# entn-at/exemplars_vc

Hardware: AMD Instinct MI355X
Metric: spectral frames/sec converted (100 NMF iters, N=4096 dict) (higher is better)
Workload: dtype f64

## Files before the change

exemplars_vc_amd/csrc/evc_fused_all.hip:

```cpp
#include "evc_fused_common.h"

namespace evc {

constexpr int AW = 4;
constexpr int AKT = 8;
constexpr int ATILES = AW * AKT;
constexpr int ATHREADS = 2 * AW * 64;
constexpr unsigned ALL_POLL_LIMIT = 1u << 17;
#ifndef EVC_ALL_STAGGER_PER_ITER
#define EVC_ALL_STAGGER_PER_ITER 11000
#endif
#ifndef EVC_ALL_EXCH_PRIO
#define EVC_ALL_EXCH_PRIO 3
#endif
#ifndef EVC_ALL_C1_ALTERNATE
#define EVC_ALL_C1_ALTERNATE 0
#endif

constexpr long ALL_LDS_BUDGET = 160 * 1024 - 256;
__host__ __device__ constexpr int all_dict_row(int e) { return 4 * (((e >> 2) & 1) * 2 + (e >> 3)) + (e & 3); }
template <int MSTEPS, int C, bool KL>
struct AllShape {
    static constexpr int MT = MSTEPS > 4 ? 2 : 1;
    static constexpr int E = MT * 4 * 64;
    static constexpr int NE = MSTEPS * 64;
    static constexpr int RSTR = NE < 256 ? 256 : NE;
    static constexpr int STG = C > 0 ? 1 : (C == 0 ? NE : NE + ALL_MAX_MEMBERS - 1);
    static constexpr long REST = 8L * 2 * (AW * RSTR + 2 * E + (KL ? E : 1) + STG) + 3 * 4;
    static constexpr long dict_bytes(int pr) { return 8L * ATILES * 16 * pr; }
    static constexpr int PR_ALL = 4 * MSTEPS + 2;
    static constexpr int PR = KL ? 0
                              : REST + dict_bytes(PR_ALL) <= ALL_LDS_BUDGET       ? PR_ALL
                              : REST + dict_bytes(PR_ALL - 4) <= ALL_LDS_BUDGET   ? PR_ALL - 4
                                                                                  : 0;
    static constexpr bool LDS_DICT = C != 1 && PR > 0 && PR - 1 >= 4 * MSTEPS - 3;
};

#ifdef EVC_ALL_TIMING
#define EVC_STAMP(i)                                                                                             \
    do {                                                                                                         \
        if (a.dbg && tt0 == g - half && lane == 0 && w == 0)                                                     \
            a.dbg[(((long)blockIdx.x * 2 + half) * (2 * a.iters + 1) + step) * 4 + (i)] = __builtin_amdgcn_s_memtime(); \
    } while (0)
#else
#define EVC_STAMP(i)
#endif

template <int MSTEPS, int C, bool KL>
__global__ __launch_bounds__(ATHREADS, 2) void k_fused_all(FusedArgs a) {
    using S = AllShape<MSTEPS, C, KL>;
    constexpr int MT = S::MT;
    constexpr int E = S::E;
    constexpr int NE = S::NE;
    constexpr int RSTR = S::RSTR;
    constexpr int MSP = (MSTEPS + 1) & ~1;
    constexpr int PR = S::PR;
    constexpr int TPD = 16 * PR;
    __shared__ double s_red[2][AW * RSTR];
    __shared__ double s_v[2][E];
    __shared__ double s_x[2][E];
    __shared__ double s_r[2][KL ? E : 1];
    __shared__ double s_stage[2][S::STG];
    __shared__ double s_dict[S::LDS_DICT ? ATILES * TPD : 1];
    __shared__ unsigned s_hb[2];
    __shared__ int s_fail;
    const int tid = threadIdx.x, lane = tid & 63;
    const int w8 = __builtin_amdgcn_readfirstlane(tid >> 6);
    const int half = w8 >> 2, w = w8 & 3, th = tid & (AW * 64 - 1);
    const int CR = C > 0 ? C : a.coop_c;
    const int member = blockIdx.x % CR;
    const int g = 2 * (blockIdx.x / CR) + half;
    double* const red = s_red[half];
    double* const vL = s_v[half];
    double* const xL = s_x[half];
    double* const rL = s_r[half];
    double* const stage = s_stage[half];
    unsigned hb = 0;
    const double* __restrict__ A1p = a.A1p;
    const double* __restrict__ A2p = a.A2p;
    f64x2* __restrict__ Hp = a.Hp;
    const int NT = a.NT;
    const long tile0 = (long)member * ATILES + w;
    const unsigned ul = (unsigned)lane;
    long sw = 0;

    const __amdgpu_buffer_rsrc_t r1 = __builtin_amdgcn_make_buffer_rsrc(const_cast<double*>(A1p), 0, NT * (MSP * 512), 0x00020000);
    const __amdgpu_buffer_rsrc_t r2 = __builtin_amdgcn_make_buffer_rsrc(const_cast<double*>(A2p), 0, NT * (MT * 2048), 0x00020000);
#ifdef EVC_ALL_NOFRAG
    bool nofrag_go = false;
#endif
    const unsigned ul16 = ul * 16u, ul8 = ul * 8u;
    constexpr int BL = 16 * ((MSTEPS - 1) >> 2) + 4 * ((MSTEPS - 1) & 3);
    const int rowA = w * AKT * TPD + all_dict_row(4 * (lane & 3) + ((lane & 15) >> 2)) * PR;
    const int rowB = w * AKT * TPD + all_dict_row(4 * (lane >> 4)) * PR;
    const double* const dA = s_dict + rowA + (lane >> 4);
    const double* const dAL = s_dict + rowA + min(lane >> 4, a.M - BL);
    const double* const dB = s_dict + rowB + (lane & 15);
    const double* const dBL = s_dict + rowB + min(lane & 15, a.M - 16 * (MT - 1));
#define LDS_NO_PAIR() asm volatile("" ::: "memory")
    auto load_a1 = [&](double (&a1)[MSTEPS], int k, auto lds) {
        if constexpr (decltype(lds)::value) {
#pragma unroll
            for (int s = 0; s < MSTEPS; ++s) {
                a1[s] = (s == MSTEPS - 1 ? dAL : dA)[k * TPD + 16 * (s >> 2) + 4 * (s & 3)];
                LDS_NO_PAIR();
            }
            return;
        }
#ifdef EVC_ALL_NOFRAG
        if (nofrag_go) return;
#endif
        const int so = (int)(tile0 + sw + AW * k) * (MSP * 512);
#pragma unroll
        for (int s = 0; s < MSTEPS; s += 2) {
            if (s + 1 < MSTEPS) {
                const f64x2 v = __builtin_bit_cast(f64x2, __builtin_amdgcn_raw_buffer_load_b128(r1, ul16 + (s >> 1) * 1024, so, 0));
                a1[s] = v[0];
                a1[s + 1] = v[1];
            } else {
                a1[s] = __builtin_bit_cast(double, __builtin_amdgcn_raw_buffer_load_b64(r1, ul16 + (s >> 1) * 1024, so, 0));
            }
        }
    };
    auto load_a2 = [&](double (&a2)[MT][4], int k, auto lds) {
        if constexpr (decltype(lds)::value) {
#pragma unroll
            for (int u = 0; u < MT; ++u)
#pragma unroll
                for (int r = 0; r < 4; ++r) {
                    a2[u][r] = (u == MT - 1 ? dBL : dB)[k * TPD + r * PR + 16 * u];
                    LDS_NO_PAIR();
                }
            return;
        }
#ifdef EVC_ALL_NOFRAG
        if (nofrag_go) return;
#endif
        const int so = (int)(tile0 + sw + AW * k) * (MT * 2048);
#pragma unroll
        for (int u = 0; u < MT; ++u)
#pragma unroll
            for (int r = 0; r < 4; r += 2) {
                const f64x2 v = __builtin_bit_cast(f64x2, __builtin_amdgcn_raw_buffer_load_b128(r2, ul16 + (u * 2 + (r >> 1)) * 1024, so, 0));
                a2[u][r] = v[0];
                a2[u][r + 1] = v[1];
            }
    };
    (void)ul8;

    const int mode = a.eps_mode;
    const double eps = a.eps;
    const double d0 = a.l1 + (mode == EVC_EPS_ADD ? a.eps : 0.0);
    const f64x4 dinit = {d0, d0, d0, d0};
    const unsigned lo = fast_lo(mode, eps);
    unsigned seq = 0;
    int rs_es = 1, rs_len = 0, rs_pub0 = 0, rs_pub1 = 0, rs_src0 = -1, rs_src1 = -1, rs_src2 = -1;
    if (C < 0) {
        rs_es = (NE + CR - 1) / CR;
        rs_len = NE - member * rs_es;
        rs_len = rs_len < 0 ? 0 : (rs_len > rs_es ? rs_es : rs_len);
        const int e0 = th, e1 = th + AW * 64;
        const int j0 = e0 / rs_es, j1 = (e1 < NE ? e1 : e0) / rs_es;
        rs_pub0 = (j0 * CR + member) * rs_es + (e0 - j0 * rs_es);
        rs_pub1 = (j1 * CR + member) * rs_es + ((e1 < NE ? e1 : e0) - j1 * rs_es);
        auto src = [&](int idx) {
            if (idx >= CR * rs_es) return -1;
            const int el = idx % rs_es;
            return el < rs_len ? member * CR * rs_es + idx : -1;
        };
        rs_src0 = src(th);
        rs_src1 = src(th + AW * 64);
        rs_src2 = src(th + 2 * AW * 64);
    }
    if (tid == 0) s_fail = 0;
    if (tid < 2) s_hb[tid] = 0;

    if (a.stagger_cycles > 0 && ((blockIdx.x / CR) & 1)) {
        const long long t0 = __builtin_amdgcn_s_memtime();
        while (__builtin_amdgcn_s_memtime() - t0 < a.stagger_cycles) __builtin_amdgcn_s_sleep(32);
    }

    auto run = [&](auto lds) __attribute__((always_inline)) {
    for (long tt0 = g - half; tt0 < a.TT; tt0 += a.groups) {
        const long tt = tt0 + half;
        bool valid;
        {
            const long t = 16 * tt + (lane & 15);
            int u = -1;
            if (tt < a.TT && t < a.T_) u = a.frame_utt[t];
            const bool live = tt < a.TT && ((t >= a.T_) || ((u >= 0) && (a.active[u] != 0)));
            const int v0 = __syncthreads_and(half == 0 ? live : true);
            const int v1 = __syncthreads_and(half == 1 ? live : true);
            valid = (half ? v1 : v0) != 0;
        }
        HTile h[AKT];
        f64x4 p[AKT];
        double a1[MSTEPS], a2[MT][4];
        if (valid && a.first && a.init_const) {
            auto h0_of = [&](int fr) {
                const long t = 16 * tt + fr;
                const int u = t < a.T_ ? a.frame_utt[t] : -1;
                return u >= 0 ? a.h0[u] : 0.0;
            };
            for (int e = th; e < E; e += AW * 64) {
                const int s = e >> 6, l = e & 63;
                const bool in = s < MSTEPS;
                xL[e] = in ? a.Xp[(tt * MSTEPS + s) * 64 + l] : 0.0;
                vL[e] = in ? a.rsum[bin_of(s, l >> 4)] * h0_of(l & 15) : 0.0;
                if (KL) rL[e] = xL[e] / (vL[e] < a.eps ? a.eps : vL[e]);
            }
            const double hv = h0_of(lane & 15);
#pragma unroll
            for (int k = 0; k < AKT; ++k) {
                const long n0 = 16 * (tile0 + AW * k) + 4 * (lane >> 4);
#pragma unroll
                for (int r = 0; r < 4; ++r) h[k][r] = n0 + r < a.N ? hv : 0.0;
            }
        } else if (valid) {
            for (int e = th; e < E; e += AW * 64) {
                const int s = e >> 6, l = e & 63;
                const bool in = s < MSTEPS;
                xL[e] = in ? a.Xp[(tt * MSTEPS + s) * 64 + l] : 0.0;
                vL[e] = in ? a.Vp[(tt * 8 + s) * 64 + l] : 0.0;
                if (KL) rL[e] = xL[e] / (vL[e] < a.eps ? a.eps : vL[e]);
            }
#pragma unroll
            for (int k = 0; k < AKT; ++k) {
                const f64x2* t = Hp + (tt * NT + tile0 + AW * k) * 128;
                const f64x2 h01 = t[ul], h23 = t[ul + 64];
                h[k][0] = h01[0]; h[k][1] = h01[1]; h[k][2] = h23[0]; h[k][3] = h23[1];
            }
        }
        __syncthreads();
        if (valid && !KL) {
            double x[MSTEPS];
#pragma unroll
            for (int s = 0; s < MSTEPS; ++s) x[s] = xL[s * 64 + lane];
            load_a1(a1, 0, lds);
#pragma unroll
            for (int k = 0; k < AKT; ++k) {
                f64x4 acc = {0, 0, 0, 0};
#pragma unroll
                for (int s = 0; s < MSTEPS; ++s) acc = Mma<double>::mma(a1[s], x[s], acc);
                if (!decltype(lds)::value || k + 1 < AKT) load_a1(a1, (k + 1) % AKT, lds);
                p[k] = acc;
            }
        }

        if (valid && KL) load_a1(a1, 0, lds);
        for (int step = 0; step <= 2 * a.iters; ++step) {
#ifdef EVC_ALL_NOFRAG
            nofrag_go = step > 2;
#endif
            const bool mine = (C == 1 && !EVC_ALL_C1_ALTERNATE) ? (step & 1) == 0 : (step & 1) == half;
            EVC_STAMP(0);
            if (valid && mine && step < 2 * a.iters) {
                asm volatile("" : "+s"(sw));
                double v[MSTEPS];
#pragma unroll
                for (int s = 0; s < MSTEPS; ++s) v[s] = KL ? rL[s * 64 + lane] : vL[s * 64 + lane];
                if constexpr (decltype(lds)::value) load_a1(a1, 0, lds);
                f64x4 vn[MT];
#pragma unroll
                for (int u = 0; u < MT; ++u) vn[u] = f64x4{0, 0, 0, 0};
#pragma unroll
                for (int k = 0; k < AKT; ++k) {
                    __builtin_amdgcn_sched_barrier(0);
                    load_a2(a2, k, lds);
                    f64x4 d = KL ? f64x4{0, 0, 0, 0} : dinit;
#pragma unroll
                    for (int s = 0; s < MSTEPS; ++s) d = Mma<double>::mma(a1[s], v[s], d);
                    if (!decltype(lds)::value || k + 1 < AKT)
                        load_a1(a1, (k + 1) % AKT, lds);
                    __builtin_amdgcn_sched_barrier(0);
                    if (KL) {
#pragma unroll
                        for (int r = 0; r < 4; ++r) h[k][r] *= d[r];
                    } else {
                        mu_tile_guarded(h[k], p[k], d, mode, eps, lo);
                    }
#pragma unroll
                    for (int u = 0; u < MT; ++u)
#pragma unroll
                        for (int r = 0; r < 4; ++r) vn[u] = Mma<double>::mma(a2[u][r], h[k][r], vn[u]);
                }
#pragma unroll
                for (int u = 0; u < MT; ++u)
#pragma unroll
                    for (int r = 0; r < 4; ++r)
                        if (u * 4 + r < MSTEPS) red[w * RSTR + (u * 4 + r) * 64 + lane] = vn[u][r];
            } else if (valid && !mine && step > 0) {
                const int e0 = C <= 0 ? th % NE : th, e1 = th + AW * 64;
                const bool has1 = e1 < NE;
                __builtin_amdgcn_s_setprio(EVC_ALL_EXCH_PRIO);
                double s0 = 0.0, s1 = 0.0;
#pragma unroll
                for (int ww = 0; ww < AW; ++ww) {
                    s0 += red[ww * RSTR + e0];
                    s1 += red[ww * RSTR + (has1 ? e1 : e0)];
                }
                if (C < 0) {
                    long long* xb1 = reinterpret_cast<long long*>(a.coop_buf) +
                                     ((size_t)(seq & 1) * a.groups + g) * (size_t)CR * ALL_RS_STRIDE;
                    long long* xb2 = reinterpret_cast<long long*>(a.coop_buf) + ALL_SLICE_OFFSET +
                                     ((size_t)(seq & 1) * a.groups + g) * 512;
                    const long long tag = (seq >> 1) & 1;
                    __hip_atomic_store(xb1 + rs_pub0, (__double_as_longlong(s0) & ~1LL) | tag, __ATOMIC_RELAXED,
                                       __HIP_MEMORY_SCOPE_AGENT);
                    if (has1)
                        __hip_atomic_store(xb1 + rs_pub1, (__double_as_longlong(s1) & ~1LL) | tag, __ATOMIC_RELAXED,
                                           __HIP_MEMORY_SCOPE_AGENT);
                    bool ok = true;
                    auto fetch3 = [&](const long long* p0, const long long* p1, const long long* p2, long long& b0,
                                      long long& b1, long long& b2) {
                        unsigned polls = 0;
                        for (;;) {
                            b0 = __hip_atomic_load(p0, __ATOMIC_RELAXED, __HIP_MEMORY_SCOPE_AGENT);
                            b1 = __hip_atomic_load(p1, __ATOMIC_RELAXED, __HIP_MEMORY_SCOPE_AGENT);
                            b2 = __hip_atomic_load(p2, __ATOMIC_RELAXED, __HIP_MEMORY_SCOPE_AGENT);
                            if (__all(!ok || (((b0 ^ tag) | (b1 ^ tag) | (b2 ^ tag)) & 1) == 0)) break;
                            if (++polls > ALL_POLL_LIMIT ||
                                ((polls & 63) == 0 &&
                                 __hip_atomic_load(a.coop_abort, __ATOMIC_RELAXED, __HIP_MEMORY_SCOPE_AGENT) != 0))
                                ok = false;
                            __builtin_amdgcn_s_sleep(1);
                        }
                    };
                    {
                        long long b0, b1, b2;
                        const long long* own = xb1 + rs_pub0;
                        fetch3(rs_src0 >= 0 ? xb1 + rs_src0 : own, rs_src1 >= 0 ? xb1 + rs_src1 : own,
                               rs_src2 >= 0 ? xb1 + rs_src2 : own, b0, b1, b2);
                        if (rs_src0 >= 0) stage[th] = __longlong_as_double(b0 & ~1LL);
                        if (rs_src1 >= 0) stage[th + AW * 64] = __longlong_as_double(b1 & ~1LL);
                        if (rs_src2 >= 0) stage[th + 2 * AW * 64] = __longlong_as_double(b2 & ~1LL);
                        hb += AW;
                        if (lane == 0)
                            __hip_atomic_fetch_add(&s_hb[half], 1u, __ATOMIC_RELEASE, __HIP_MEMORY_SCOPE_WORKGROUP);
                        while ((int)(__hip_atomic_load(&s_hb[half], __ATOMIC_ACQUIRE, __HIP_MEMORY_SCOPE_WORKGROUP) - hb) < 0)
                            __builtin_amdgcn_s_sleep(1);
                        const int q = th & 3;
                        for (int el = th >> 2; el < rs_len; el += AW * 16) {
                            double v = 0.0;
                            for (int m = q; m < CR; m += 4) v += stage[m * rs_es + el];
                            v += __shfl_xor(v, 1, 64);
                            v += __shfl_xor(v, 2, 64);
                            if (q == 0)
                                __hip_atomic_store(xb2 + member * rs_es + el, (__double_as_longlong(v) & ~1LL) | tag,
                                                   __ATOMIC_RELAXED, __HIP_MEMORY_SCOPE_AGENT);
                        }
                    }
                    long long g0, g1, g2;
                    fetch3(xb2 + e0, xb2 + (has1 ? e1 : e0), xb2 + e0, g0, g1, g2);
                    s0 = __longlong_as_double(g0 & ~1LL);
                    s1 = __longlong_as_double(g1 & ~1LL);
                    ++seq;
                    if (!ok) s_fail = 1;
                } else if (C == 0) {
                    const int ES = NE / CR;
                    long long* xb1 = reinterpret_cast<long long*>(a.coop_buf) +
                                     ((size_t)(seq & 1) * a.groups + g) * (size_t)CR * 512;
                    long long* xb2 = reinterpret_cast<long long*>(a.coop_buf) + ALL_SLICE_OFFSET +
                                     ((size_t)(seq & 1) * a.groups + g) * 512;
                    const long long tag = (seq >> 1) & 1;
                    {
                        const int j0 = e0 / ES, j1 = (has1 ? e1 : e0) / ES;
                        __hip_atomic_store(xb1 + ((size_t)j0 * CR + member) * ES + (e0 - j0 * ES),
                                           (__double_as_longlong(s0) & ~1LL) | tag, __ATOMIC_RELAXED,
                                           __HIP_MEMORY_SCOPE_AGENT);
                        if (has1)
                            __hip_atomic_store(xb1 + ((size_t)j1 * CR + member) * ES + (e1 - j1 * ES),
                                               (__double_as_longlong(s1) & ~1LL) | tag, __ATOMIC_RELAXED,
                                               __HIP_MEMORY_SCOPE_AGENT);
                    }
                    bool ok = true;
                    auto fetch2 = [&](const long long* p0, const long long* p1, long long& b0, long long& b1) {
                        unsigned polls = 0;
                        for (;;) {
                            b0 = __hip_atomic_load(p0, __ATOMIC_RELAXED, __HIP_MEMORY_SCOPE_AGENT);
                            b1 = __hip_atomic_load(p1, __ATOMIC_RELAXED, __HIP_MEMORY_SCOPE_AGENT);
                            if (__all(!ok || (((b0 ^ tag) | (b1 ^ tag)) & 1) == 0)) break;
                            if (++polls > ALL_POLL_LIMIT ||
                                ((polls & 63) == 0 &&
                                 __hip_atomic_load(a.coop_abort, __ATOMIC_RELAXED, __HIP_MEMORY_SCOPE_AGENT) != 0))
                                ok = false;
                            __builtin_amdgcn_s_sleep(1);
                        }
                    };
                    {
                        long long b0, b1;
                        const long long* mine_ = xb1 + (size_t)member * NE;
                        fetch2(mine_ + e0, mine_ + (has1 ? e1 : e0), b0, b1);
                        stage[e0] = __longlong_as_double(b0 & ~1LL);
                        if (has1) stage[e1] = __longlong_as_double(b1 & ~1LL);
                        hb += AW;
                        if (lane == 0)
                            __hip_atomic_fetch_add(&s_hb[half], 1u, __ATOMIC_RELEASE, __HIP_MEMORY_SCOPE_WORKGROUP);
                        while ((int)(__hip_atomic_load(&s_hb[half], __ATOMIC_ACQUIRE, __HIP_MEMORY_SCOPE_WORKGROUP) - hb) < 0)
                            __builtin_amdgcn_s_sleep(1);
                        if (th < 4 * ES) {
                            const int el = th >> 2, q = th & 3, per = CR >> 2;
                            double v = 0.0;
                            for (int i = 0; i < per; ++i) v += stage[(q * per + i) * ES + el];
                            v += __shfl_xor(v, 1, 64);
                            v += __shfl_xor(v, 2, 64);
                            if (q == 0)
                                __hip_atomic_store(xb2 + member * ES + el, (__double_as_longlong(v) & ~1LL) | tag,
                                                   __ATOMIC_RELAXED, __HIP_MEMORY_SCOPE_AGENT);
                        }
                    }
                    long long g0, g1;
                    fetch2(xb2 + e0, xb2 + (has1 ? e1 : e0), g0, g1);
                    s0 = __longlong_as_double(g0 & ~1LL);
                    s1 = __longlong_as_double(g1 & ~1LL);
                    ++seq;
                    if (!ok) s_fail = 1;
                } else if (C > 1) {
                    long long* xb = reinterpret_cast<long long*>(a.coop_buf) +
                                    ((size_t)(seq & 1) * a.groups + g) * (size_t)(C * 512);
                    const long long tag = (seq >> 1) & 1;
                    const long long m0 = (__double_as_longlong(s0) & ~1LL) | tag;
                    const long long m1 = (__double_as_longlong(s1) & ~1LL) | tag;
                    __hip_atomic_store(xb + member * 512 + e0, m0, __ATOMIC_RELAXED, __HIP_MEMORY_SCOPE_AGENT);
                    if (has1) __hip_atomic_store(xb + member * 512 + e1, m1, __ATOMIC_RELAXED, __HIP_MEMORY_SCOPE_AGENT);
                    bool ok = true;
                    unsigned polls = 0;
                    {
                        const long long* sp = xb + (lane < C ? lane : 0) * 512 + (NE - 1);
                        for (;;) {
                            const long long b = __hip_atomic_load(sp, __ATOMIC_RELAXED, __HIP_MEMORY_SCOPE_AGENT);
                            const bool ready = lane >= C || lane == member || (b & 1) == tag;
                            if (__all(ready)) break;
                            if (++polls > ALL_POLL_LIMIT ||
                                ((polls & 63) == 0 &&
                                 __hip_atomic_load(a.coop_abort, __ATOMIC_RELAXED, __HIP_MEMORY_SCOPE_AGENT) != 0)) {
                                ok = false;
                                break;
                            }
                            __builtin_amdgcn_s_sleep(2);
                        }
                    }
                    long long b0[C > 0 ? C : 1] = {}, b1[C > 0 ? C : 1] = {};
                    polls = 0;
                    while (ok) {
#pragma unroll
                        for (int m = 0; m < C; ++m)
                            b0[m] = __hip_atomic_load(xb + m * 512 + e0, __ATOMIC_RELAXED, __HIP_MEMORY_SCOPE_AGENT);
#pragma unroll
                        for (int m = 0; m < C; ++m)
                            b1[m] = __hip_atomic_load(xb + m * 512 + (has1 ? e1 : e0), __ATOMIC_RELAXED, __HIP_MEMORY_SCOPE_AGENT);
                        long long bad = 0;
#pragma unroll
                        for (int m = 0; m < C; ++m) {
                            b0[m] = (m == member) ? m0 : b0[m];
                            b1[m] = (m == member) ? m1 : b1[m];
                            bad |= (b0[m] ^ tag) | (b1[m] ^ tag);
                        }
                        if ((bad & 1) == 0) break;
                        if (++polls > ALL_POLL_LIMIT ||
                            ((polls & 63) == 0 &&
                             __hip_atomic_load(a.coop_abort, __ATOMIC_RELAXED, __HIP_MEMORY_SCOPE_AGENT) != 0)) {
                            ok = false;
                            break;
                        }
                        __builtin_amdgcn_s_sleep(2);
                    }
                    s0 = 0.0; s1 = 0.0;
#pragma unroll
                    for (int m = 0; m < C; ++m) {
                        s0 += __longlong_as_double(b0[m] & ~1LL);
                        s1 += __longlong_as_double(b1[m] & ~1LL);
                    }
                    ++seq;
                    if (!ok) s_fail = 1;
                }
                vL[e0] = s0;
                if (has1) vL[e1] = s1;
                if (KL) {
                    rL[e0] = xL[e0] / (s0 < a.eps ? a.eps : s0);
                    if (has1) rL[e1] = xL[e1] / (s1 < a.eps ? a.eps : s1);
                }
                __builtin_amdgcn_s_setprio(0);
            }
            EVC_STAMP(1);
            __syncthreads();
            EVC_STAMP(2);
            if (C != 1 && s_fail) {
                if (tid == 0) __hip_atomic_store(a.coop_abort, 1, __ATOMIC_RELAXED, __HIP_MEMORY_SCOPE_AGENT);
                return;
            }
        }

        if (valid) {
#pragma unroll
            for (int k = 0; k < AKT; ++k) {
                f64x2* t = Hp + (tt * NT + tile0 + AW * k) * 128;
                t[ul] = f64x2{h[k][0], h[k][1]};
                t[ul + 64] = f64x2{h[k][2], h[k][3]};
            }
            if (a.Hx) {
                const long t = 16 * tt + (lane & 15);
                if (t < a.T_) {
#pragma unroll
                    for (int k = 0; k < AKT; ++k) {
                        const long n0 = 16 * (tile0 + AW * k) + 4 * (lane >> 4);
#pragma unroll
                        for (int r = 0; r < 4; ++r)
                            if (n0 + r < a.N) {
                                if (a.hx_frame_major) a.Hx[t * a.ldhx + n0 + r] = h[k][r];
                                else a.Hx[(n0 + r) * a.ldhx + t] = h[k][r];
                            }
                    }
                }
            }
            if (member == 0) {
                for (int e = th; e < NE; e += AW * 64) a.Vp[(tt * 8 + (e >> 6)) * 64 + (e & 63)] = vL[e];
                if (a.write_err && w == 0) {
                    double e = 0.0;
#pragma unroll
                    for (int s = 0; s < MSTEPS; ++s) {
                        const double x = xL[s * 64 + lane], vv = vL[s * 64 + lane];
                        e += KL ? kl_terms(x, vv, a.eps) : (x - vv) * (x - vv);
                    }
                    e += __shfl_xor(e, 16, 64);
                    e += __shfl_xor(e, 32, 64);
                    const long t = 16 * tt + lane;
                    if (lane < 16 && t < a.T_) a.err2[t] = e;
                }
            }
        }
        __syncthreads();
    }
    };

    if constexpr (S::LDS_DICT) {
        if (a.M > 0 && a.M < PR) {
            for (int x = tid; x < ATILES * TPD; x += ATHREADS) {
                const int slot = x / TPD, e = all_dict_row((x / PR) % 16), b = x % PR;
                const long j = (long)member * ATILES + slot / AKT + AW * (slot % AKT);
                const int q = e >> 2, r = e & 3;
                s_dict[x] = b < a.M ? A2p[((j * MT + (b >> 4)) * 2 + (r >> 1)) * 128 + (16 * q + (b & 15)) * 2 + (r & 1)] : 0.0;
            }
            __syncthreads();
            run(std::true_type{});
            return;
        }
    }
    run(std::false_type{});
}

template <int MSTEPS, int C, bool KL>
static hipError_t launch_all(FusedArgs a, int n_cus, hipStream_t s) {
    int occ = 0;
    hipError_t e = hipOccupancyMaxActiveBlocksPerMultiprocessor(&occ, k_fused_all<MSTEPS, C, KL>, ATHREADS, 0);
    if (e != hipSuccess) return e;
    if (occ < 1) return hipErrorInvalidValue;
    long resident = n_cus;
    if (2 * resident > ALL_MAX_WGS) resident = ALL_MAX_WGS / 2;
    const int cr = C > 0 ? C : a.coop_c;
    if (C == 0 && (cr < 8 || cr > 64 || (cr & (cr - 1)))) return hipErrorInvalidValue;
    if (C < 0 && (cr < 2 || cr > ALL_MAX_MEMBERS)) return hipErrorInvalidValue;
    int pairs = (int)(resident / cr);
    const int want = (a.TT + 1) / 2;
    if (pairs > want) pairs = want;
    if (pairs < 1) return hipErrorInvalidValue;
    a.groups = 2 * pairs;
    a.stagger_cycles = (a.iters > 0 && a.iters <= 25 && a.TT >= 4L * a.groups && pairs >= 2) ? (long long)a.iters * EVC_ALL_STAGGER_PER_ITER : 0;
    if (C != 1) {
        e = hipMemsetAsync(a.coop_buf, 0xFF, sizeof(double) * 2 * (size_t)a.groups * cr * (C < 0 ? ALL_RS_STRIDE : 512), s);
        if (e != hipSuccess) return e;
    }
    if (C <= 0) {
        if (2L * a.groups * 512 > ALL_SLICE_ELEMS) return hipErrorInvalidValue;
        e = hipMemsetAsync(a.coop_buf + ALL_SLICE_OFFSET, 0xFF, sizeof(double) * 2 * (size_t)a.groups * 512, s);
        if (e != hipSuccess) return e;
    }
    hipLaunchKernelGGL((k_fused_all<MSTEPS, C, KL>), dim3((unsigned)(pairs * cr)), dim3(ATHREADS), 0, s, a);
    return hipGetLastError();
}

template <int MSTEPS, bool KL>
static hipError_t pick_c(const FusedArgs& a, int n_cus, hipStream_t s) {
    switch (a.NT / ATILES) {
        case 1: return launch_all<MSTEPS, 1, KL>(a, n_cus, s);
        case 2: return launch_all<MSTEPS, 2, KL>(a, n_cus, s);
        case 4: return launch_all<MSTEPS, 4, KL>(a, n_cus, s);
        case 8:
            if constexpr (AllShape<MSTEPS, 8, KL>::LDS_DICT)
                if (a.M > 0 && a.M < AllShape<MSTEPS, 8, KL>::PR) return launch_all<MSTEPS, 8, KL>(a, n_cus, s);
            return launch_all<MSTEPS, 0, KL>(a, n_cus, s);
        case 16:
        case 32:
        case 64: return launch_all<MSTEPS, 0, KL>(a, n_cus, s);
        default: return launch_all<MSTEPS, -1, KL>(a, n_cus, s);
    }
}

int fused_all_members(int NT, int N, int eps_mode, int exact_div, int loss) {
    if (eps_mode == EVC_EPS_NONE || exact_div || (loss != EVC_LOSS_FROBENIUS && loss != EVC_LOSS_KL)) return 0;
    if (NT % ATILES) return 0;
    const int c = NT / ATILES;
    if (loss == EVC_LOSS_KL && c >= 2 && c < 16) return 0;
    return (c >= 1 && c <= ALL_MAX_MEMBERS) ? c : 0;
}

hipError_t fused_all_launch(int msteps, const FusedArgs& a, int n_cus, hipStream_t s) {
    if (a.NT % ATILES || !a.coop_buf || !a.coop_abort) return hipErrorInvalidValue;
    switch (msteps) {
        case 1: return a.loss == EVC_LOSS_KL ? pick_c<1, true>(a, n_cus, s) : pick_c<1, false>(a, n_cus, s);
        case 2: return a.loss == EVC_LOSS_KL ? pick_c<2, true>(a, n_cus, s) : pick_c<2, false>(a, n_cus, s);
        case 3: return a.loss == EVC_LOSS_KL ? pick_c<3, true>(a, n_cus, s) : pick_c<3, false>(a, n_cus, s);
        case 4: return a.loss == EVC_LOSS_KL ? pick_c<4, true>(a, n_cus, s) : pick_c<4, false>(a, n_cus, s);
        case 5: return a.loss == EVC_LOSS_KL ? pick_c<5, true>(a, n_cus, s) : pick_c<5, false>(a, n_cus, s);
        case 6: return a.loss == EVC_LOSS_KL ? pick_c<6, true>(a, n_cus, s) : pick_c<6, false>(a, n_cus, s);
        case 7: return a.loss == EVC_LOSS_KL ? pick_c<7, true>(a, n_cus, s) : pick_c<7, false>(a, n_cus, s);
        case 8: return a.loss == EVC_LOSS_KL ? pick_c<8, true>(a, n_cus, s) : pick_c<8, false>(a, n_cus, s);
        default: return hipErrorInvalidValue;
    }
}

}
```

Baseline: 1.096 million.

## Restructure cross-block reduction polling and move failure check before barrier

Replaces the two-phase cooperative exchange wait (first spin on a sentinel element, then reload every member's data) with a single loop. Each peer's values are fetched directly, and only peers that have not yet arrived are re-polled, tracked in a bitmask. The failure flag becomes double-buffered per step parity and is read before the barrier, so the post-barrier shared-memory check and the extra serialization it caused go away. It also adds tunable fetch-delay and retry-sleep macros and extra timing stamps; the trade-off is more complex abort semantics, where the early return depends on the previous step's flag.

```diff
diff --git a/exemplars_vc_amd/csrc/evc_fused_all.hip b/exemplars_vc_amd/csrc/evc_fused_all.hip
--- a/exemplars_vc_amd/csrc/evc_fused_all.hip
+++ b/exemplars_vc_amd/csrc/evc_fused_all.hip
@@ -15,6 +15,12 @@
 #endif
 #ifndef EVC_ALL_C1_ALTERNATE
 #define EVC_ALL_C1_ALTERNATE 0
+#endif
+#ifndef EVC_ALL_FETCH_DELAY
+#define EVC_ALL_FETCH_DELAY 0
+#endif
+#ifndef EVC_ALL_RETRY_SLEEP
+#define EVC_ALL_RETRY_SLEEP 2
 #endif
 
 constexpr long ALL_LDS_BUDGET = 160 * 1024 - 256;
@@ -40,7 +46,7 @@
 #define EVC_STAMP(i)                                                                                             \
     do {                                                                                                         \
         if (a.dbg && tt0 == g - half && lane == 0 && w == 0)                                                     \
-            a.dbg[(((long)blockIdx.x * 2 + half) * (2 * a.iters + 1) + step) * 4 + (i)] = __builtin_amdgcn_s_memtime(); \
+            a.dbg[(((long)blockIdx.x * 2 + half) * (2 * a.iters + 1) + step) * 8 + (i)] = __builtin_amdgcn_s_memtime(); \
     } while (0)
 #else
 #define EVC_STAMP(i)
@@ -63,7 +69,7 @@
     __shared__ double s_stage[2][S::STG];
     __shared__ double s_dict[S::LDS_DICT ? ATILES * TPD : 1];
     __shared__ unsigned s_hb[2];
-    __shared__ int s_fail;
+    __shared__ int s_fail[2];
     const int tid = threadIdx.x, lane = tid & 63;
     const int w8 = __builtin_amdgcn_readfirstlane(tid >> 6);
     const int half = w8 >> 2, w = w8 & 3, th = tid & (AW * 64 - 1);
@@ -172,13 +178,18 @@
         rs_src1 = src(th + AW * 64);
         rs_src2 = src(th + 2 * AW * 64);
     }
-    if (tid == 0) s_fail = 0;
+    if (tid < 2) s_fail[tid] = 0;
     if (tid < 2) s_hb[tid] = 0;
 
     if (a.stagger_cycles > 0 && ((blockIdx.x / CR) & 1)) {
         const long long t0 = __builtin_amdgcn_s_memtime();
         while (__builtin_amdgcn_s_memtime() - t0 < a.stagger_cycles) __builtin_amdgcn_s_sleep(32);
     }
+
+    auto give_up = [&](int step) {
+        __hip_atomic_store(a.coop_abort, 1, __ATOMIC_RELAXED, __HIP_MEMORY_SCOPE_AGENT);
+        s_fail[step & 1] = 1;
+    };
 
     auto run = [&](auto lds) __attribute__((always_inline)) {
     for (long tt0 = g - half; tt0 < a.TT; tt0 += a.groups) {
@@ -254,6 +265,12 @@
 #endif
             const bool mine = (C == 1 && !EVC_ALL_C1_ALTERNATE) ? (step & 1) == 0 : (step & 1) == half;
             EVC_STAMP(0);
+            int failed = 0;
+            if (C != 1) {
+                int slot = (step + 1) & 1;
+                asm volatile("" : "+v"(slot));
+                failed = __hip_atomic_load(&s_fail[slot], __ATOMIC_RELAXED, __HIP_MEMORY_SCOPE_WORKGROUP);
+            }
             if (valid && mine && step < 2 * a.iters) {
                 asm volatile("" : "+s"(sw));
                 double v[MSTEPS];
@@ -355,7 +372,7 @@
                     s0 = __longlong_as_double(g0 & ~1LL);
                     s1 = __longlong_as_double(g1 & ~1LL);
                     ++seq;
-                    if (!ok) s_fail = 1;
+                    if (!ok) give_up(step);
                 } else if (C == 0) {
                     const int ES = NE / CR;
                     long long* xb1 = reinterpret_cast<long long*>(a.coop_buf) +
@@ -414,7 +431,7 @@
                     s0 = __longlong_as_double(g0 & ~1LL);
                     s1 = __longlong_as_double(g1 & ~1LL);
                     ++seq;
-                    if (!ok) s_fail = 1;
+                    if (!ok) give_up(step);
                 } else if (C > 1) {
                     long long* xb = reinterpret_cast<long long*>(a.coop_buf) +
                                     ((size_t)(seq & 1) * a.groups + g) * (size_t)(C * 512);
@@ -423,47 +440,50 @@
                     const long long m1 = (__double_as_longlong(s1) & ~1LL) | tag;
                     __hip_atomic_store(xb + member * 512 + e0, m0, __ATOMIC_RELAXED, __HIP_MEMORY_SCOPE_AGENT);
                     if (has1) __hip_atomic_store(xb + member * 512 + e1, m1, __ATOMIC_RELAXED, __HIP_MEMORY_SCOPE_AGENT);
+                    EVC_STAMP(3);
+                    long long b0[C > 0 ? C : 1] = {}, b1[C > 0 ? C : 1] = {};
+                    const long long* const q0 = xb + e0;
+                    const long long* const q1 = xb + (has1 ? e1 : e0);
+                    const unsigned tagw = (unsigned)tag;
+                    unsigned need = ((1u << C) - 1u) & ~(1u << member);
                     bool ok = true;
                     unsigned polls = 0;
-                    {
-                        const long long* sp = xb + (lane < C ? lane : 0) * 512 + (NE - 1);
-                        for (;;) {
-                            const long long b = __hip_atomic_load(sp, __ATOMIC_RELAXED, __HIP_MEMORY_SCOPE_AGENT);
-                            const bool ready = lane >= C || lane == member || (b & 1) == tag;
-                            if (__all(ready)) break;
-                            if (++polls > ALL_POLL_LIMIT ||
-                                ((polls & 63) == 0 &&
-                                 __hip_atomic_load(a.coop_abort, __ATOMIC_RELAXED, __HIP_MEMORY_SCOPE_AGENT) != 0)) {
-                                ok = false;
-                                break;
-                            }
-                            __builtin_amdgcn_s_sleep(2);
-                        }
-                    }
-                    long long b0[C > 0 ? C : 1] = {}, b1[C > 0 ? C : 1] = {};
-                    polls = 0;
-                    while (ok) {
-#pragma unroll
-                        for (int m = 0; m < C; ++m)
-                            b0[m] = __hip_atomic_load(xb + m * 512 + e0, __ATOMIC_RELAXED, __HIP_MEMORY_SCOPE_AGENT);
-#pragma unroll
-                        for (int m = 0; m < C; ++m)
-                            b1[m] = __hip_atomic_load(xb + m * 512 + (has1 ? e1 : e0), __ATOMIC_RELAXED, __HIP_MEMORY_SCOPE_AGENT);
-                        long long bad = 0;
-#pragma unroll
-                        for (int m = 0; m < C; ++m) {
-                            b0[m] = (m == member) ? m0 : b0[m];
-                            b1[m] = (m == member) ? m1 : b1[m];
-                            bad |= (b0[m] ^ tag) | (b1[m] ^ tag);
-                        }
-                        if ((bad & 1) == 0) break;
+                    auto fetch = [&](int m) {
+                        b0[m] = __hip_atomic_load(q0 + m * 512, __ATOMIC_RELAXED, __HIP_MEMORY_SCOPE_AGENT);
+                        b1[m] = __hip_atomic_load(q1 + m * 512, __ATOMIC_RELAXED, __HIP_MEMORY_SCOPE_AGENT);
+                    };
+                    auto arrived = [&](int m) {
+                        const bool late = ((((unsigned)b0[m] ^ tagw) | ((unsigned)b1[m] ^ tagw)) & 1u) != 0;
+                        return __builtin_amdgcn_ballot_w64(late) == 0;
+                    };
+                    if (EVC_ALL_FETCH_DELAY > 0) __builtin_amdgcn_s_sleep(EVC_ALL_FETCH_DELAY);
+#pragma unroll
+                    for (int m = 0; m < C; ++m)
+                        if (m != member) fetch(m);
+#pragma unroll
+                    for (int m = 0; m < C; ++m)
+                        if (m != member && arrived(m)) need &= ~(1u << m);
+                    EVC_STAMP(4);
+                    while (need != 0) {
                         if (++polls > ALL_POLL_LIMIT ||
                             ((polls & 63) == 0 &&
                              __hip_atomic_load(a.coop_abort, __ATOMIC_RELAXED, __HIP_MEMORY_SCOPE_AGENT) != 0)) {
                             ok = false;
                             break;
                         }
-                        __builtin_amdgcn_s_sleep(2);
+                        __builtin_amdgcn_s_sleep(EVC_ALL_RETRY_SLEEP);
+#pragma unroll
+                        for (int m = 0; m < C; ++m)
+                            if ((need >> m) & 1) fetch(m);
+#pragma unroll
+                        for (int m = 0; m < C; ++m)
+                            if (((need >> m) & 1) && arrived(m)) need &= ~(1u << m);
+                    }
+                    EVC_STAMP(5);
+#pragma unroll
+                    for (int m = 0; m < C; ++m) {
+                        b0[m] = (m == member) ? m0 : b0[m];
+                        b1[m] = (m == member) ? m1 : b1[m];
                     }
                     s0 = 0.0; s1 = 0.0;
 #pragma unroll
@@ -472,7 +492,7 @@
                         s1 += __longlong_as_double(b1[m] & ~1LL);
                     }
                     ++seq;
-                    if (!ok) s_fail = 1;
+                    if (!ok) give_up(step);
                 }
                 vL[e0] = s0;
                 if (has1) vL[e1] = s1;
@@ -483,12 +503,9 @@
                 __builtin_amdgcn_s_setprio(0);
             }
             EVC_STAMP(1);
+            if (C != 1 && __builtin_amdgcn_readfirstlane(failed)) return;
             __syncthreads();
             EVC_STAMP(2);
-            if (C != 1 && s_fail) {
-                if (tid == 0) __hip_atomic_store(a.coop_abort, 1, __ATOMIC_RELAXED, __HIP_MEMORY_SCOPE_AGENT);
-                return;
-            }
         }
 
         if (valid) {
```

Measured after the change: 1.106 million, median of 6. Within noise of the previous version (+1.0%).

## Exchange cross-block partial sums with 128-bit buffer stores and tag-checked polling

Applied to the files above, without the earlier changes.

Adds a new exchange path for fixed cooperative group sizes (C>1). Each thread now reduces two adjacent partials and publishes them with a single 16-byte buffer store carrying a parity tag bit. It then waits on the last element of each peer slot before doing vectorized 128-bit loads of all peers' data, retrying until every tag matches. The aim is fewer memory transactions and less polling in the inter-workgroup reduction. The cost is a new alignment requirement on coop_buf and a reliance on 16-byte stores being observed atomically, with the watch loop only sampling the final element.

```diff
diff --git a/exemplars_vc_amd/csrc/evc_fused_all.hip b/exemplars_vc_amd/csrc/evc_fused_all.hip
--- a/exemplars_vc_amd/csrc/evc_fused_all.hip
+++ b/exemplars_vc_amd/csrc/evc_fused_all.hip
@@ -16,6 +16,14 @@
 #ifndef EVC_ALL_C1_ALTERNATE
 #define EVC_ALL_C1_ALTERNATE 0
 #endif
+#ifndef EVC_ALL_X16
+#define EVC_ALL_X16 1
+#endif
+#ifndef EVC_ALL_X16_WATCH
+#define EVC_ALL_X16_WATCH 1
+#endif
+typedef unsigned all_u32x4 __attribute__((ext_vector_type(4)));
+typedef long long all_i64x2 __attribute__((ext_vector_type(2)));
 
 constexpr long ALL_LDS_BUDGET = 160 * 1024 - 256;
 __host__ __device__ constexpr int all_dict_row(int e) { return 4 * (((e >> 2) & 1) * 2 + (e >> 3)) + (e & 3); }
@@ -56,10 +64,10 @@
     constexpr int MSP = (MSTEPS + 1) & ~1;
     constexpr int PR = S::PR;
     constexpr int TPD = 16 * PR;
-    __shared__ double s_red[2][AW * RSTR];
-    __shared__ double s_v[2][E];
-    __shared__ double s_x[2][E];
-    __shared__ double s_r[2][KL ? E : 1];
+    __shared__ __attribute__((aligned(16))) double s_red[2][AW * RSTR];
+    __shared__ __attribute__((aligned(16))) double s_v[2][E];
+    __shared__ __attribute__((aligned(16))) double s_x[2][E];
+    __shared__ __attribute__((aligned(16))) double s_r[2][KL ? E : 1];
     __shared__ double s_stage[2][S::STG];
     __shared__ double s_dict[S::LDS_DICT ? ATILES * TPD : 1];
     __shared__ unsigned s_hb[2];
@@ -86,6 +94,7 @@
 
     const __amdgpu_buffer_rsrc_t r1 = __builtin_amdgcn_make_buffer_rsrc(const_cast<double*>(A1p), 0, NT * (MSP * 512), 0x00020000);
     const __amdgpu_buffer_rsrc_t r2 = __builtin_amdgcn_make_buffer_rsrc(const_cast<double*>(A2p), 0, NT * (MT * 2048), 0x00020000);
+    const __amdgpu_buffer_rsrc_t rx = __builtin_amdgcn_make_buffer_rsrc(a.coop_buf, 0, C > 1 ? 2 * a.groups * (C * 4096) : 0, 0x00020000);
 #ifdef EVC_ALL_NOFRAG
     bool nofrag_go = false;
 #endif
@@ -289,6 +298,88 @@
 #pragma unroll
                     for (int r = 0; r < 4; ++r)
                         if (u * 4 + r < MSTEPS) red[w * RSTR + (u * 4 + r) * 64 + lane] = vn[u][r];
+            } else if (C > 1 && EVC_ALL_X16 && valid && !mine && step > 0) {
+                __builtin_amdgcn_s_setprio(EVC_ALL_EXCH_PRIO);
+                const bool act = th < NE / 2;
+                const int ep = act ? 2 * th : 0;
+                f64x2 sm = {0.0, 0.0};
+                if (w * 64 < NE / 2) {
+                    f64x2 pv[AW];
+#pragma unroll
+                    for (int ww = 0; ww < AW; ++ww) pv[ww] = *reinterpret_cast<const f64x2*>(red + ww * RSTR + ep);
+                    static_assert(AW == 4, "the four partials are named one by one");
+                    asm volatile("" : "+v"(pv[0]), "+v"(pv[1]), "+v"(pv[2]), "+v"(pv[3]));
+#pragma unroll
+                    for (int ww = 0; ww < AW; ++ww) sm += pv[ww];
+                    const long long tag = (seq >> 1) & 1;
+                    const long long m0 = (__double_as_longlong(sm[0]) & ~1LL) | tag;
+                    const long long m1 = (__double_as_longlong(sm[1]) & ~1LL) | tag;
+                    const int xo = __builtin_amdgcn_readfirstlane((int)(((seq & 1) * (unsigned)a.groups + (unsigned)g) * (unsigned)(C * 4096)));
+                    if (act)
+                        __builtin_amdgcn_raw_buffer_store_b128(__builtin_bit_cast(all_u32x4, all_i64x2{m0, m1}), rx, ep * 8,
+                                                               xo + member * 4096, 16);
+                    bool ok = true;
+                    unsigned polls = 0;
+#if EVC_ALL_X16_WATCH
+                    {
+                        const long long* sp = reinterpret_cast<const long long*>(a.coop_buf) +
+                                              ((size_t)(seq & 1) * a.groups + g) * (size_t)(C * 512) +
+                                              (lane < C ? lane : 0) * 512 + (NE - 1);
+                        for (;;) {
+                            const long long b = __hip_atomic_load(sp, __ATOMIC_RELAXED, __HIP_MEMORY_SCOPE_AGENT);
+                            const bool ready = lane >= C || lane == member || (b & 1) == tag;
+                            if (__all(ready)) break;
+                            if (++polls > ALL_POLL_LIMIT ||
+                                ((polls & 63) == 0 &&
+                                 __hip_atomic_load(a.coop_abort, __ATOMIC_RELAXED, __HIP_MEMORY_SCOPE_AGENT) != 0)) {
+                                ok = false;
+                                break;
+                            }
+                            __builtin_amdgcn_s_sleep(2);
+                        }
+                    }
+#endif
+                    all_i64x2 b[C > 0 ? C : 1] = {};
+                    polls = 0;
+                    while (__builtin_expect(ok && act, 1)) {
+                        asm volatile("" ::: "memory");
+#pragma unroll
+                        for (int m = 0; m < C; ++m)
+                            if (m != member)
+                                b[m] = __builtin_bit_cast(all_i64x2, __builtin_amdgcn_raw_buffer_load_b128(rx, ep * 8, xo + m * 4096, 16));
+                        long long bad = 0;
+#pragma unroll
+                        for (int m = 0; m < C; ++m) {
+                            b[m] = (m == member) ? all_i64x2{m0, m1} : b[m];
+                            bad |= (b[m][0] ^ tag) | (b[m][1] ^ tag);
+                        }
+                        if ((bad & 1) == 0) break;
+                        if (++polls > ALL_POLL_LIMIT ||
+                            ((polls & 63) == 0 &&
+                             __hip_atomic_load(a.coop_abort, __ATOMIC_RELAXED, __HIP_MEMORY_SCOPE_AGENT) != 0)) {
+                            ok = false;
+                            break;
+                        }
+                        __builtin_amdgcn_s_sleep(2);
+                    }
+                    f64x2 v2 = {0.0, 0.0};
+#pragma unroll
+                    for (int m = 0; m < C; ++m) {
+                        v2[0] += __longlong_as_double(b[m][0] & ~1LL);
+                        v2[1] += __longlong_as_double(b[m][1] & ~1LL);
+                    }
+                    if (!ok) s_fail = 1;
+                    if (act) {
+                        *reinterpret_cast<f64x2*>(vL + ep) = v2;
+                        if (KL) {
+                            const f64x2 x2 = *reinterpret_cast<const f64x2*>(xL + ep);
+                            *reinterpret_cast<f64x2*>(rL + ep) =
+                                f64x2{x2[0] / (v2[0] < a.eps ? a.eps : v2[0]), x2[1] / (v2[1] < a.eps ? a.eps : v2[1])};
+                        }
+                    }
+                }
+                ++seq;
+                __builtin_amdgcn_s_setprio(0);
             } else if (valid && !mine && step > 0) {
                 const int e0 = C <= 0 ? th % NE : th, e1 = th + AW * 64;
                 const bool has1 = e1 < NE;
@@ -566,6 +657,7 @@
     if (pairs < 1) return hipErrorInvalidValue;
     a.groups = 2 * pairs;
     a.stagger_cycles = (a.iters > 0 && a.iters <= 25 && a.TT >= 4L * a.groups && pairs >= 2) ? (long long)a.iters * EVC_ALL_STAGGER_PER_ITER : 0;
+    if (C > 1 && (reinterpret_cast<uintptr_t>(a.coop_buf) & 15)) return hipErrorInvalidValue;
     if (C != 1) {
         e = hipMemsetAsync(a.coop_buf, 0xFF, sizeof(double) * 2 * (size_t)a.groups * cr * (C < 0 ? ALL_RS_STRIDE : 512), s);
         if (e != hipSuccess) return e;
```

After: 1.103 million before, 1.116 million after, median of 6. 1.01x the previous value.
